# scrose/pylc

Measured on AMD Instinct MI355X. Metric: 512x512 tiles/sec fwd+bwd (DeepLabV3+/ResNet101, 9-class), higher is better.
Workload: dtype f32; 1 GPU; DeepLabV3+ ResNet101 OS16, 3-ch 512x512 tiles, 9 classes, CE+Dice+Focal, clip 0.5 + AdamW, bs=32/GPU (BASELINE.json configs[2]); global_batch=32, parallelism=dp1, conv_arithmetic=f16x3 split (fp32-grade), rccl_ranks=0, wgrad_queue=compute stream, sync_bn=True, activation_format=fp16 planes between BatchNorm and conv kernels (4 B/element)

## Files before the change

### include/pylc_hip.h

```cpp
#ifndef PYLC_HIP_H
#define PYLC_HIP_H

#include <stddef.h>
#include <stdint.h>

#ifdef __cplusplus
extern "C" {
#endif

#define PYLC_OK 0
#define PYLC_ERR_ARG 1
#define PYLC_ERR_HIP 2
#define PYLC_ERR_WORKSPACE 3
#define PYLC_ERR_UNSUPPORTED 4

const char* pylc_last_error(void);
int pylc_abi_version(void);
int pylc_experimental_build(void);
int pylc_init(void);

typedef struct PylcConvDesc {
    int B, H, W;
    int Cin, Cout;
    int R, S;
// ... 85 lines not shown
} PylcBnBack;
size_t pylc_conv2d_dgrad_bn_floats(const PylcConvDesc* d);
int pylc_conv2d_dgrad_bn(const PylcConvDesc* d, const float* dy, const float* w_crsk, float* dx, int accumulate,
                         const float* add_src, const void* add_mask, const PylcBnBack* bn, float* sums_partial, int* sums_rows,
                         void* stream);
#endif
int pylc_relu_bwd_bits(const float* dout, const void* mask, float* g_out, long long M, int C, void* stream);
int pylc_conv2d_dgrad_needs_f32_weights(const PylcConvDesc* d);
size_t pylc_conv2d_wgrad_workspace(const PylcConvDesc* d);
int pylc_conv2d_wgrad(const PylcConvDesc* d, const float* x, const float* dy, float* dw_krsc,
                      float* dbias ,
                      void* workspace, size_t workspace_bytes, void* stream);
typedef struct PylcSlabSum {
    const float* slabs;
    float* dw;
    long long n4;
    long long slab_stride;
    int splits;
    int reserved;
} PylcSlabSum;
int pylc_conv2d_wgrad_slabs(const PylcConvDesc* d, const float* x, const float* dy, float* dw_krsc, void* workspace, size_t workspace_bytes,
                            PylcSlabSum* pending, void* stream);
int pylc_splitk_reduce_batch(const PylcSlabSum* table_dev, const long long* tile_prefix_dev, int n, long long total_tiles, void* stream);
int pylc_weight_transpose(const float* w_krsc, float* w_crsk, int K, int RS, int C, void* stream);

typedef struct PylcDwDesc {
    int B, H, W, C;
    int stride, dil;
    int OH, OW;
    int x_pitch, y_pitch;
} PylcDwDesc;
int pylc_dwconv3x3_fwd(const PylcDwDesc* d, const float* x, const float* w, float* y, void* stream);
int pylc_dwconv3x3_fwd_stats_rows(const PylcDwDesc* d);
int pylc_dwconv3x3_fwd_stats(const PylcDwDesc* d, const float* x, const float* w_c9, float* y, float* stats_partial, void* stream);
int pylc_dwconv3x3_dgrad(const PylcDwDesc* d, const float* dy, const float* w, float* dx, void* stream);
int pylc_dwconv3x3_dgrad_acc(const PylcDwDesc* d, const float* dy, const float* w_c9, float* dx, int accumulate, void* stream);
size_t pylc_dwconv3x3_wgrad_workspace(const PylcDwDesc* d);
int pylc_dwconv3x3_wgrad(const PylcDwDesc* d, const float* x, const float* dy, float* dw,
                         void* workspace, size_t workspace_bytes, void* stream);
int pylc_dwconv3x3_half_ok(const PylcDwDesc* d);
int pylc_dwconv3x3_fwd_h_stats_rows(const PylcDwDesc* d);
int pylc_dwconv3x3_fwd_h(const PylcDwDesc* d, const void* x_h, const unsigned int* x_bound, const float* w_c9, const unsigned int* w_amax,
                         void* y_h, unsigned int* y_bound_out, float* stats_partial, void* stream);
int pylc_dwconv3x3_fwd_h_eval(const PylcDwDesc* d, const void* x_h, const unsigned int* x_bound, const unsigned int* x_true_amax, const float* w,
                              const unsigned int* w_amax, void* y_h, unsigned int* y_bound_out, void* stream);
int pylc_dwconv3x3_dgrad_h(const PylcDwDesc* d, const void* dy_h, const unsigned int* dy_bound, const float* w_c9, const unsigned int* w_amax,
// ... 283 lines not shown
```

### pylc_amd/csrc/conv_common.h

```cpp
#pragma once
#include "common.h"
#include <type_traits>

namespace pylc {

typedef float f32x4 __attribute__((ext_vector_type(4)));
typedef float f32x16 __attribute__((ext_vector_type(16)));

typedef __bf16 bf16x8 __attribute__((ext_vector_type(8)));

typedef _Float16 f16x8 __attribute__((ext_vector_type(8)));
typedef _Float16 f16x2 __attribute__((ext_vector_type(2)));
typedef float f32x2 __attribute__((ext_vector_type(2)));

constexpr int LDB = 80;

__device__ __forceinline__ void split3(const float (&x)[4], uint2& p0, uint2& p1, uint2& p2) {
    unsigned u0[4], u1[4], u2[4];
#pragma unroll
    for (int e = 0; e < 4; ++e) {
        u0[e] = __float_as_uint(x[e]);
        const float r1 = x[e] - __uint_as_float(u0[e] & 0xFFFF0000u);
        u1[e] = __float_as_uint(r1);
        const float r2 = r1 - __uint_as_float(u1[e] & 0xFFFF0000u);
// ... 130 lines not shown
    const unsigned* amax_x;
    long long x_bytes, dy_bytes;
    const void* x_planes;
    const void* dy_planes;
    long long x_plane_stride, dy_plane_stride;
    int nterms;
    int dbg_flags;
};

typedef short s16x4 __attribute__((ext_vector_type(4)));
typedef short s16x8 __attribute__((ext_vector_type(8)));
typedef s16x4 __attribute__((address_space(3))) * lds_s16x4_ptr;

__host__ __device__ constexpr int wg_rowb(int w) { return w * 2 + (w == 32 ? 0 : 64); }

__device__ __forceinline__ bf16x8 tr_frag(const char* p, int rowb) {
    const s16x4 lo = __builtin_amdgcn_ds_read_tr16_b64_v4i16((lds_s16x4_ptr)(p));
    const s16x4 hi = __builtin_amdgcn_ds_read_tr16_b64_v4i16((lds_s16x4_ptr)(p + 4 * rowb));
    const s16x8 v = __builtin_shufflevector(lo, hi, 0, 1, 2, 3, 4, 5, 6, 7);
    return __builtin_bit_cast(bf16x8, v);
}


int launch_wg_pl(WgradArgs& a, int cfg, long long grid, hipStream_t st);
int wgrad_pl_init();

bool takes_pl(const GatherGemmArgs& a);
int launch_gg_pl(GatherGemmArgs& a, hipStream_t st);
int conv_pl_init();
bool takes_stem(const GatherGemmArgs& a);
int launch_stem_fwd(GatherGemmArgs& a, hipStream_t st);
int conv_stem_init();

extern int g_conv_precision;
extern int g_wg_flags;
extern int g_pp_flags;

}
```

### pylc_amd/csrc/conv_igemm.hip

```cpp
#include "conv_common.h"

namespace pylc {

template <int BM, int BN, int WM, int WN, bool CIN4, int PREC>
__global__ __launch_bounds__((BM / WM) * (BN / WN) * 64, 2) void gather_gemm_kernel(const GatherGemmArgs a) {
    constexpr int WAVES_N = BN / WN;
    constexpr int MT = WM / 32, NT = WN / 32;
    constexpr int NTHR = (BM / WM) * (BN / WN) * 64;
    constexpr int RPI = NTHR / 8;
    constexpr int A_IT = BM / RPI, B_IT = BN / RPI;
    static_assert(NTHR == 256 || NTHR == 512, "4 or 8 waves per block");
    static_assert(BM % RPI == 0 && BN % RPI == 0, "tile rows must divide evenly over the loader");
    extern __shared__ __attribute__((aligned(16))) float smem[];
    float* sA = smem;
    float* sB = smem + 2 * BM * LDT;

    const int tile = xcd_remap(blockIdx.x, gridDim.x);
    const int m0 = (tile / a.tiles_n) * BM;
    const int n0 = (tile % a.tiles_n) * BN;
    const int tid = threadIdx.x, lane = tid & 63, wave = tid >> 6;
    const int wave_m = wave / WAVES_N, wave_n = wave % WAVES_N;
    const int v = tid & 7, r0 = tid >> 3;

    int rowh[A_IT], roww[A_IT], rowpix[A_IT];
// ... 1878 lines not shown

extern "C" int pylc_splitk_reduce_batch(const PylcSlabSum* table_dev, const long long* tile_prefix_dev, int n, long long total_tiles, void* stream) {
    PYLC_REQUIRE(table_dev && tile_prefix_dev && n > 0 && total_tiles > 0, "splitk_reduce_batch: bad arguments");
    const int blocks = (int)(total_tiles < 4096 ? total_tiles : 4096);
    hipLaunchKernelGGL(splitk_reduce_batch_kernel, dim3(blocks), dim3(256), 0, as_stream(stream), table_dev, tile_prefix_dev, n, total_tiles);
    PYLC_LAUNCH_CHECK();
    return PYLC_OK;
}

static int wgrad_impl(const PylcConvDesc* d, const float* x, const float* dy, float* dw, float* dbias,
                      void* workspace, size_t workspace_bytes, PylcSlabSum* pending, void* stream);

extern "C" int pylc_conv2d_wgrad(const PylcConvDesc* d, const float* x, const float* dy, float* dw, float* dbias,
                                 void* workspace, size_t workspace_bytes, void* stream) {
    return wgrad_impl(d, x, dy, dw, dbias, workspace, workspace_bytes, nullptr, stream);
}

extern "C" int pylc_conv2d_wgrad_slabs(const PylcConvDesc* d, const float* x, const float* dy, float* dw, void* workspace, size_t workspace_bytes,
                                       PylcSlabSum* pending, void* stream) {
    PYLC_REQUIRE(pending != nullptr, "conv2d_wgrad_slabs: null `pending`");
    return wgrad_impl(d, x, dy, dw, nullptr, workspace, workspace_bytes, pending, stream);
}

static int wgrad_impl(const PylcConvDesc* d, const float* x, const float* dy, float* dw, float* dbias,
                      void* workspace, size_t workspace_bytes, PylcSlabSum* pending, void* stream) {
    if (int rc = check_desc(d)) return rc;
    PYLC_REQUIRE(x && dy && dw, "null pointer");
    PYLC_REQUIRE(dbias == nullptr, "dbias: use pylc_bn_stats on dy (column sums)");
    PYLC_REQUIRE(d->x_fmt == d->dy_fmt, "conv2d_wgrad: x and dy must be in the same format (both fp32 or both fp16 planes; pylc_to_planes converts)");
    hipStream_t st = as_stream(stream);
    const WgradPlan p = plan_wgrad(d);
    const size_t need = p.splits > 1 ? (size_t)p.splits * p.slab * sizeof(float) : 0;
    if (need > workspace_bytes || (need && !workspace))
        return fail(PYLC_ERR_WORKSPACE, "wgrad workspace too small: need %zu bytes, got %zu", need, workspace_bytes);
    PYLC_REQUIRE(p.slab % 4 == 0, "dw size must be a multiple of 4");
    const int T = d->R * d->S;
    WgradArgs a{};
    a.x = x; a.dy = dy; a.out = p.splits > 1 ? static_cast<float*>(workspace) : dw;
    a.P = d->OH; a.Q = d->OW; a.M = d->B * d->OH * d->OW;
    a.IH = d->H; a.IW = d->W; a.Cin = d->Cin; a.x_pitch = d->x_pitch; a.in_sh = a.in_sw = d->stride;
    a.TR = d->R; a.TS = d->S; a.dh0 = -d->pad; a.dh_step = d->dil; a.dw0 = -d->pad; a.dw_step = d->dil;
    a.N = d->Cout; a.N_ld = roundup4(d->Cout); a.dy_pitch = d->y_pitch;
    PYLC_REQUIRE(a.N_ld <= d->y_pitch, "dy pitch must cover roundup4(Cout)");
    a.out_row_stride = T * d->Cin;
    a.tiles_n = p.tiles_n; a.tiles_c = p.tiles_c; a.splits = p.splits; a.m_per_split = p.m_per_split;
    a.slab_stride = p.slab;
    PYLC_REQUIRE(g_conv_precision < 2 || (d->dy_amax && d->x_amax), "f16x3 / fp16 mode: conv2d_wgrad needs dy_amax and x_amax in the descriptor");
    a.x_bytes = (((long long)d->B * d->H * d->W - 1) * d->x_pitch + d->Cin) * 4;
    a.dy_bytes = (((long long)d->B * d->OH * d->OW - 1) * d->y_pitch + a.N_ld) * 4;
    a.amax_dy = d->dy_amax; a.amax_x = d->x_amax;
    const long long grid = (long long)p.tiles_n * p.tiles_c * (p.cin4 ? 1 : T) * p.splits;
    int rc;
    if (d->x_fmt == 1) {
        PYLC_REQUIRE(g_conv_precision >= 2 && !p.cin4 && d->Cout % 8 == 0, "conv2d_wgrad: fp16-plane operands need precision mode 2 or 3, "
                     "a dense geometry and Cout %% 8 == 0");
        a.x_planes = x; a.dy_planes = dy; a.x = nullptr; a.dy = nullptr;
        a.x_plane_stride = planes_stride_rule((long long)d->B * d->H * d->W, d->Cin, d->x_pitch, (g_conv_precision == 3 ? 1 : 2));
        a.dy_plane_stride = planes_stride_rule((long long)d->B * d->OH * d->OW, d->Cout, d->y_pitch, (g_conv_precision == 3 ? 1 : 2));
        a.N_ld = d->Cout;
        a.x_bytes /= 2; a.dy_bytes = (((long long)d->B * d->OH * d->OW - 1) * d->y_pitch + a.N_ld) * 2;
        a.nterms = g_conv_precision == 3 ? 1 : 3;
        rc = launch_wg_pl(a, p.cfg, grid, st);
    } else
    switch (p.cfg) {
        case 0: rc = launch_wg<128, 128, 64, 64, false>(a, grid, st); break;
        case 1: rc = launch_wg<64, 64, 32, 32, false>(a, grid, st); break;
        case 2: rc = launch_wg<32, 128, 32, 32, false>(a, grid, st); break;
        default: rc = launch_wg<64, 64, 32, 32, true>(a, grid, st); break;
    }
    if (rc) return rc;
    if (pending != nullptr) {
        *pending = PylcSlabSum{p.splits > 1 ? static_cast<const float*>(workspace) : nullptr, dw, p.slab / 4, p.slab, p.splits > 1 ? p.splits : 0, 0};
        return PYLC_OK;
    }
    if (p.splits > 1) {
        const long long n4 = p.slab / 4;
        const int blocks = (int)(cdiv<long long>(n4, 32) < 4096 ? cdiv<long long>(n4, 32) : 4096);
        hipLaunchKernelGGL(splitk_reduce_kernel, dim3(blocks), dim3(256), 0, st, static_cast<const float*>(workspace), dw, n4,
                           p.splits, p.slab);
        PYLC_LAUNCH_CHECK();
    }
    return PYLC_OK;
}

extern "C" int pylc_weight_transpose(const float* w, float* wt, int K, int RS, int C, void* stream) {
    PYLC_REQUIRE(w && wt && K > 0 && RS > 0 && C > 0, "bad weight_transpose arguments");
    const int Kp = roundup4(K);
    dim3 grid(cdiv(C, 32), cdiv(Kp, 32), RS);
    hipLaunchKernelGGL(weight_transpose_kernel, grid, dim3(256), 0, as_stream(stream), w, wt, K, RS, C, Kp);
    PYLC_LAUNCH_CHECK();
    return PYLC_OK;
}
```

### pylc_amd/csrc/wgrad_pl.hip

```cpp
#include "conv_common.h"

namespace pylc {

typedef __attribute__((address_space(3))) void* wg_lds_vptr;
template <int BN, int BC, int WN, int WC, int NTERMS, int FAST, bool ACC1 = false, int SETS = 1, bool M16 = false, bool DMA = false>
__global__ __launch_bounds__(256, ACC1 ? 4 : 2) void wgrad_pl_kernel(const WgradArgs a) {
    static_assert(!DMA || (M16 && SETS == 1), "DMA: the 16x16x32 image only");
    constexpr int NPL = NTERMS == 3 ? 2 : 1;
    constexpr int WAVES_C = BC / WC;
    constexpr int NT = WN / 32, CT = WC / 32;
    static_assert(!M16 || (BN == 128 && BC == 128 && WN == 64 && WC == 64 && !ACC1), "M16: 128 x 128 block tiles, 64 x 64 wave tiles, two accumulator sets");
    constexpr int VA = BN / 8, RA = 256 / VA, IA = 32 / RA > 0 ? 32 / RA : 1;
    constexpr int VB = BC / 8, RB = 256 / VB, IB = 32 / RB > 0 ? 32 / RB : 1;
    constexpr bool A_ALL = RA <= 32, B_ALL = RB <= 32;
    constexpr int ROWA = M16 ? 256 : wg_rowb(BN), ROWB = M16 ? 256 : wg_rowb(BC);
    constexpr int PLA = 32 * ROWA, PLB = 32 * ROWB;
    static_assert((BN / WN) * (BC / WC) == 4, "4 waves per block");
    static_assert(FAST == 1 || FAST == 2, "buffer-load geometry paths only");
    extern __shared__ __attribute__((aligned(16))) float smem[];
    char* sA = reinterpret_cast<char*>(smem);
    char* sB = sA + NPL * PLA;
    constexpr int STG = NPL * (PLA + PLB);

    const int T = a.TR * a.TS;
    int id = (a.dbg_flags & 1) ? (int)blockIdx.x : xcd_remap(blockIdx.x, gridDim.x);
    int tc, tn, tap, split;
    if (a.dbg_flags & 2) {
        split = id % a.splits; id /= a.splits;
        tc = id % a.tiles_c; id /= a.tiles_c;
        tn = id % a.tiles_n; id /= a.tiles_n;
        tap = id;
    } else if (a.dbg_flags & 4) {
        tc = id % a.tiles_c; id /= a.tiles_c;
        tn = id % a.tiles_n; id /= a.tiles_n;
        tap = id % T; id /= T;
        split = id;
    } else if (a.Cin > a.N && !(a.dbg_flags & 8)) {
        tap = id % T; id /= T;
        tn = id % a.tiles_n; id /= a.tiles_n;
        tc = id % a.tiles_c; id /= a.tiles_c;
        split = id;
    } else {
        tap = id % T; id /= T;
        tc = id % a.tiles_c; id /= a.tiles_c;
        tn = id % a.tiles_n; id /= a.tiles_n;
        split = id;
    }
    const int n0 = tn * BN, c0 = tc * BC;
// ... 382 lines not shown
                    if (n < a.N) out[(size_t)n * a.out_row_stride + col_base + c] = val;
                }
        }
        return;
    }
#pragma unroll
    for (int j = 0; j < CT; ++j) {
        const int c = c0 + wave_c * WC + j * 32 + (lane & 31);
        if (c >= a.Cin) continue;
#pragma unroll
        for (int i = 0; i < NT; ++i) {
#pragma unroll
            for (int r = 0; r < 16; ++r) {
                const int n = n0 + wave_n * WN + i * 32 + (r & 3) + 8 * (r >> 2) + 4 * (lane >> 5);
                float val = acc[i][j][r];
                if constexpr (TWO_ACC) val = (val + acc_lo[i][j][r] * (1.f / 2048.f)) * unscale_a * unscale_b;
                else val = val * unscale_a * unscale_b;
                if (n < a.N) out[(size_t)n * a.out_row_stride + col_base + c] = val;
            }
        }
    }
}

template <int BN, int BC, int NTERMS>
constexpr size_t wgpl_smem() { return (size_t)(NTERMS == 3 ? 2 : 1) * 32 * (wg_rowb(BN) + wg_rowb(BC)); }

int g_wg_flags = 0;
extern "C" int pylc_debug_wgrad_flags(int flags) { g_wg_flags = flags; return PYLC_OK; }
int g_wg_m16 = 2;
extern "C" int pylc_debug_wgrad_m16(int on) { g_wg_m16 = on; return PYLC_OK; }
int g_wg_dma = 1;
extern "C" int pylc_debug_wgrad_dma(int on) { g_wg_dma = on; return PYLC_OK; }
int g_wg_sets = 1;
extern "C" int pylc_debug_wgrad_sets(int mode) { g_wg_sets = mode; return PYLC_OK; }
int g_wg_acc1 = 0;
extern "C" int pylc_debug_wgrad_acc1(int on) { g_wg_acc1 = on; return PYLC_OK; }
constexpr size_t kAcc1LdsReserve = 72 * 1024;

template <int BN, int BC, int WN, int WC>
static int launch_cfg(const WgradArgs& a, long long grid, hipStream_t st) {
    const int fast = a.Q % 32 == 0 ? 1 : 2;
    const dim3 g((unsigned)grid), b(256);
    if constexpr (BN == 128 && BC == 128) {
        if (a.nterms == 3 && g_wg_acc1) {
            if (fast == 1) hipLaunchKernelGGL((wgrad_pl_kernel<BN, BC, WN, WC, 3, 1, true>), g, b, kAcc1LdsReserve, st, a);
            else hipLaunchKernelGGL((wgrad_pl_kernel<BN, BC, WN, WC, 3, 2, true>), g, b, kAcc1LdsReserve, st, a);
// ... 37 lines not shown
            if (fast == 1) hipLaunchKernelGGL((wgrad_pl_kernel<BN, BC, WN, WC, 3, 1, false, 2>), g, b, lds, st, a);
            else hipLaunchKernelGGL((wgrad_pl_kernel<BN, BC, WN, WC, 3, 2, false, 2>), g, b, lds, st, a);
        } else if (fast == 1) hipLaunchKernelGGL((wgrad_pl_kernel<BN, BC, WN, WC, 3, 1>), g, b, lds, st, a);
        else hipLaunchKernelGGL((wgrad_pl_kernel<BN, BC, WN, WC, 3, 2>), g, b, lds, st, a);
    }
    PYLC_LAUNCH_CHECK();
    return PYLC_OK;
}

int launch_wg_pl(WgradArgs& a, int cfg, long long grid, hipStream_t st) {
    a.dbg_flags = g_wg_flags;
    PYLC_REQUIRE(grid > 0 && grid < (1ll << 31), "wgrad grid out of range");
    PYLC_REQUIRE(a.x_planes && a.dy_planes && a.amax_dy && a.amax_x, "wgrad (fp16-plane operands): null planes / ranges");
    PYLC_REQUIRE(a.Q >= 16 && a.Cin % 8 == 0 && a.N_ld % 8 == 0 && a.x_pitch % 8 == 0 && a.dy_pitch % 8 == 0,
                 "wgrad (fp16-plane operands): needs OW >= 16 and channel counts / pitches that are multiples of 8");
    PYLC_REQUIRE(a.x_bytes < 0xFFFFFFF0ll && a.dy_bytes < 0xFFFFFFF0ll, "wgrad (fp16-plane operands): a plane must stay below 4 GiB");
    switch (cfg) {
        case 0: return launch_cfg<128, 128, 64, 64>(a, grid, st);
        case 1: return launch_cfg<64, 64, 32, 32>(a, grid, st);
        default: return launch_cfg<32, 128, 32, 32>(a, grid, st);
    }
}

template <typename K>
static hipError_t opt_in(K kernel, size_t bytes) {
    return hipFuncSetAttribute(reinterpret_cast<const void*>(kernel), hipFuncAttributeMaxDynamicSharedMemorySize, (int)bytes);
}

int wgrad_pl_init() {
#define PYLC_OPT(BN, BC, WN, WC)                                                                      \
    PYLC_HIP(opt_in(wgrad_pl_kernel<BN, BC, WN, WC, 3, 1>, wgpl_smem<BN, BC, 3>()));                  \
    PYLC_HIP(opt_in(wgrad_pl_kernel<BN, BC, WN, WC, 3, 2>, wgpl_smem<BN, BC, 3>()));                  \
    PYLC_HIP(opt_in(wgrad_pl_kernel<BN, BC, WN, WC, 1, 1>, wgpl_smem<BN, BC, 1>()));                  \
    PYLC_HIP(opt_in(wgrad_pl_kernel<BN, BC, WN, WC, 1, 2>, wgpl_smem<BN, BC, 1>()));                  \
    PYLC_HIP(opt_in((wgrad_pl_kernel<BN, BC, WN, WC, 3, 1, false, 2>), wgpl_smem<BN, BC, 3>()));      \
    PYLC_HIP(opt_in((wgrad_pl_kernel<BN, BC, WN, WC, 3, 2, false, 2>), wgpl_smem<BN, BC, 3>()));      \
    PYLC_HIP(opt_in((wgrad_pl_kernel<BN, BC, WN, WC, 1, 1, false, 2>), wgpl_smem<BN, BC, 1>()));      \
    PYLC_HIP(opt_in((wgrad_pl_kernel<BN, BC, WN, WC, 1, 2, false, 2>), wgpl_smem<BN, BC, 1>()));
    PYLC_OPT(128, 128, 64, 64)
    PYLC_HIP(opt_in((wgrad_pl_kernel<128, 128, 64, 64, 3, 1, false, 1, true, true>), 2 * 4 * 32 * 256));
    PYLC_HIP(opt_in((wgrad_pl_kernel<128, 128, 64, 64, 3, 2, false, 1, true, true>), 2 * 4 * 32 * 256));
    PYLC_HIP(opt_in(wgrad_pl_kernel<128, 128, 64, 64, 3, 1, true>, kAcc1LdsReserve));
    PYLC_HIP(opt_in(wgrad_pl_kernel<128, 128, 64, 64, 3, 2, true>, kAcc1LdsReserve));
    PYLC_OPT(64, 64, 32, 32)
    PYLC_OPT(32, 128, 32, 32)
#undef PYLC_OPT
    return PYLC_OK;
}

}
```

### pylc_amd/lib.py

```python
import ctypes as C
import os

import torch

_HERE = os.path.dirname(os.path.abspath(__file__))
LIB_PATH = os.environ.get('PYLC_LIB') or os.path.join(_HERE, 'libpylc_hip.so')

ABI_VERSION = 15


class PylcError(RuntimeError):
    pass


class ConvDesc(C.Structure):
    _fields_ = [(n, C.c_int) for n in ('B', 'H', 'W', 'Cin', 'Cout', 'R', 'S', 'stride', 'pad', 'dil',
                                       'OH', 'OW', 'x_pitch', 'y_pitch')] + \
               [(n, C.c_void_p) for n in ('x_amax', 'w_amax', 'dy_amax',
                                          'w_planes', 'w_planes_t')] + \
               [(n, C.c_int) for n in ('x_fmt', 'dy_fmt', 'out_fmt')] + [('out_bound', C.c_void_p)] + \
               [('w_planes_fmt', C.c_int)]


class WPrepEntry(C.Structure):
# ... 73 lines not shown
    'pylc_amax': (_I, [_P, _LL, _I, _I, _P, _P]),
    'pylc_amax_segments': (_I, [_P, _P, _I, _P, _P]),
    'pylc_to_planes': (_I, [_P, _I, _P, _I, _LL, _LL, _I, _P, _I, _P]),
    'pylc_from_planes': (_I, [_P, _I, _LL, _P, _I, _LL, _I, _P, _I, _P]),
    'pylc_planes_colsum_workspace_floats': (C.c_size_t, [_I]),
    'pylc_planes_colsum': (_I, [_P, _I, _LL, _I, _P, _LL, _I, _P, _P, _P]),
    'pylc_weight_prepare': (_I, [_P, _P, _I, _LL, _P, _P, _I, _P]),
    'pylc_conv2d_dgrad_needs_f32_weights': (_I, [C.POINTER(ConvDesc)]),
    'pylc_conv2d_fwd': (_I, [C.POINTER(ConvDesc), _P, _P, _P, _P, _P]),
    'pylc_conv2d_fwd_bnact': (_I, [C.POINTER(ConvDesc), _P, _P, _P, _P, _P, _P, _I, _P, _P, _P]),
    'pylc_conv2d_fwd_bnact_ex': (_I, [C.POINTER(ConvDesc), _P, _P, _P, C.POINTER(FwdEp), _P, _P]),
    'pylc_conv2d_fwd_stats_floats': (_SZ, [C.POINTER(ConvDesc)]),
    'pylc_conv2d_fwd_stats': (_I, [C.POINTER(ConvDesc), _P, _P, _P, _P, _P, C.POINTER(_I), _P]),
    'pylc_conv2d_dgrad': (_I, [C.POINTER(ConvDesc), _P, _P, _P, _I, _P]),
    'pylc_conv2d_dgrad_add': (_I, [C.POINTER(ConvDesc), _P, _P, _P, _I, _P, _P, _P]),
    'pylc_relu_bwd_bits': (_I, [_P, _P, _P, _LL, _I, _P]),
    'pylc_conv2d_dgrad_bn_floats': (_SZ, [C.POINTER(ConvDesc)]),
    'pylc_conv2d_dgrad_bn': (_I, [C.POINTER(ConvDesc), _P, _P, _P, _I, _P, _P, C.POINTER(BnBack), _P, C.POINTER(_I), _P]),
    'pylc_bn_bwd_sums_from_partial': (_I, [_P, _I, _I, _P, _P, _P, _D, _P, _P, _P]),
    'pylc_conv2d_wgrad_workspace': (_SZ, [C.POINTER(ConvDesc)]),
    'pylc_conv2d_wgrad': (_I, [C.POINTER(ConvDesc), _P, _P, _P, _P, _P, _SZ, _P]),
    'pylc_conv2d_wgrad_slabs': (_I, [C.POINTER(ConvDesc), _P, _P, _P, _P, _SZ, C.POINTER(SlabSum), _P]),
    'pylc_splitk_reduce_batch': (_I, [_P, _P, _I, C.c_longlong, _P]),
    'pylc_weight_transpose': (_I, [_P, _P, _I, _I, _I, _P]),
    'pylc_dwconv3x3_fwd': (_I, [C.POINTER(DwDesc), _P, _P, _P, _P]),
    'pylc_dwconv3x3_fwd_stats_rows': (_I, [C.POINTER(DwDesc)]),
    'pylc_dwconv3x3_fwd_stats': (_I, [C.POINTER(DwDesc), _P, _P, _P, _P, _P]),
    'pylc_dwconv3x3_dgrad': (_I, [C.POINTER(DwDesc), _P, _P, _P, _P]),
    'pylc_dwconv3x3_dgrad_acc': (_I, [C.POINTER(DwDesc), _P, _P, _P, _I, _P]),
    'pylc_dwconv3x3_wgrad_workspace': (_SZ, [C.POINTER(DwDesc)]),
    'pylc_dwconv3x3_wgrad': (_I, [C.POINTER(DwDesc), _P, _P, _P, _P, _SZ, _P]),
    'pylc_dwconv3x3_half_ok': (_I, [C.POINTER(DwDesc)]),
    'pylc_dwconv3x3_fwd_h_stats_rows': (_I, [C.POINTER(DwDesc)]),
    'pylc_dwconv3x3_bn_ok': (_I, [C.POINTER(DwDesc)]),
    'pylc_dwconv3x3_fwd_h_bn': (_I, [C.POINTER(DwDesc), _P, _P, _P, _P, _I, _P, _P, _P, _P, _P, _P, _P]),
    'pylc_dwconv3x3_wgrad_h_bn': (_I, [C.POINTER(DwDesc), _P, _P, _P, _P, _I, _P, _P, _P, _P, _P, _SZ, _P]),
    'pylc_dwconv3x3_dgrad_h_add_ok': (_I, [C.POINTER(DwDesc)]),
    'pylc_dwconv3x3_dgrad_h_add': (_I, [C.POINTER(DwDesc), _P, _P, _P, _P, _P, _P, _P, _P]),
    'pylc_dwconv3x3_fwd_h': (_I, [C.POINTER(DwDesc), _P, _P, _P, _P, _P, _P, _P, _P]),
    'pylc_dwconv3x3_fwd_h_eval': (_I, [C.POINTER(DwDesc), _P, _P, _P, _P, _P, _P, _P, _P]),
    'pylc_dwconv3x3_dgrad_h': (_I, [C.POINTER(DwDesc), _P, _P, _P, _P, _P, _P, _I, _P, _P]),
    'pylc_dwconv3x3_wgrad_h': (_I, [C.POINTER(DwDesc), _P, _P, _P, _P, _P, _P, _SZ, _P]),
    'pylc_bn_workspace_floats': (_SZ, [_LL, _I]),
    'pylc_bn_stats': (_I, [_P, _LL, _I, _I, _P, _P, _P]),
    'pylc_bn_stats_from_partial': (_I, [_P, _I, _I, _P, _P]),
    'pylc_bn_finalize': (_I, [_P, _D, _I, _P, _P, _F, _F, _I, _P, _P, _P, _P, _P, _P, _P]),
# ... 161 lines not shown
```

### pylc_amd/ops/_core.py

```python
import ctypes as C

import os
import time
from collections import OrderedDict
import torch
import torch.distributed as dist

from .. import lib as L
from ..lib import lib, check, ptr, stream, ConvDesc, DwDesc
from ..runtime import runtime as _runtime


def empty_nhwc(b, c, h, w, device, pitch=None, dtype=torch.float32):
    pitch = c if pitch is None else pitch
    t = torch.empty((b, h, w, pitch), device=device, dtype=dtype).permute(0, 3, 1, 2)
    return t if pitch == c else t[:, :c]


def zeros_nhwc(b, c, h, w, device, pitch=None):
    pitch = c if pitch is None else pitch
    t = torch.zeros((b, h, w, pitch), device=device, dtype=torch.float32).permute(0, 3, 1, 2)
    return t if pitch == c else t[:, :c]


# ... 332 lines not shown
    if not torch.device(device).type == 'cuda':
        return None
    return _side_streams.get(torch.device(device).index)


_side_keep = {}


def _keep_for_side(device, *tensors):
    keep = _side_keep.setdefault(torch.device(device).index, [])
    keep.extend(t for t in tensors if t is not None)
    if len(keep) > 8192:
        sync_side_streams()


_pending_slab_sums = {}
_slab_tables = {}
SLAB_TABLES_MAX = 16


_slab_callback = {}


def add_slab_sum(device, entry):
    idx = torch.device(device).index
    _pending_slab_sums.setdefault(idx, []).append(bytes(entry))
    if idx not in _slab_callback:
        st = torch.cuda.current_stream(idx)

        def at_end_of_backward(idx=idx, st=st):
            _slab_callback.pop(idx, None)
            if _pending_slab_sums.get(idx):
                with torch.cuda.stream(st):
                    flush_slab_sums(torch.device('cuda', idx))
        try:
            torch.autograd.Variable._execution_engine.queue_callback(at_end_of_backward)
            _slab_callback[idx] = st
        except RuntimeError:
            pass


def slab_sum_pending(device, workspace):
    pend = _pending_slab_sums.get(torch.device(device).index)
    if not pend:
        return False
    p = workspace.data_ptr()
    return any(L.SlabSum.from_buffer_copy(e).slabs == p for e in pend)


def reset_slab_sums():
    for pend in _pending_slab_sums.values():
        pend.clear()
    _slab_callback.clear()


def flush_slab_sums(device=None):
    for idx in ([torch.device(device).index] if device is not None else list(_pending_slab_sums)):
        pend = _pending_slab_sums.get(idx)
        if not pend:
            continue
        key = b''.join(pend)
        pend.clear()
        tables = _slab_tables.setdefault(idx, OrderedDict())
        cached = tables.get(key)
        if cached is None:
            n = len(key) // C.sizeof(L.SlabSum)
            ents = (L.SlabSum * n).from_buffer_copy(key)
            prefix = [0]
            for e in ents:
                prefix.append(prefix[-1] + (e.n4 + 31) // 32)
            dev = torch.device('cuda', idx)
            tab_h = torch.frombuffer(bytearray(key), dtype=torch.uint8).pin_memory()
            pre_h = torch.tensor(prefix, dtype=torch.int64).pin_memory()
            cached = tables[key] = (tab_h.to(dev, non_blocking=True), pre_h.to(dev, non_blocking=True), n, prefix[-1], tab_h, pre_h)
            while len(tables) > SLAB_TABLES_MAX:
                tables.popitem(last=False)
        else:
            tables.move_to_end(key)
        with torch.cuda.device(idx):
# ... 163 lines not shown
```

### pylc_amd/ops/conv.py

```python
from . import _core
from ._core import *


def _padded_stem_filter(w, cin):
    arena = getattr(w, '_pylc_arena', None)
    arena = arena() if arena is not None else None
    key = (w._version, arena.generation if arena is not None else -1, cin)
    cache = getattr(w, '_pylc_w4', None)
    if cache is not None and cache[0] == key:
        return cache[1]
    cout, cin_w, r, s = w.shape
    w_k = torch.zeros((cout, r, s, cin), device=w.device, dtype=torch.float32)
    w_k[..., :cin_w] = w.detach().permute(0, 2, 3, 1)
    w._pylc_w4 = (key, w_k)
    return w_k


class Conv2dFn(torch.autograd.Function):

    @staticmethod
    def forward(ctx, x, w, bias, stride, pad, dil, want_stats=False, x_amax=None, w_amax=None, res_link=None, out=None, convert=False, bn_src=None):
        L.init()
        ctx.set_materialize_grads(False)
        ctx.res_link = res_link if (res_link is not None and ctx.needs_input_grad[0]) else None
# ... 192 lines not shown
                mark_planes(dx, dx_bound)
            if link is not None:
                link.pending -= 1
                if link.pending > 0:
                    link.buf, dx = dx, None
                else:
                    link.buf = None
        if ctx.needs_input_grad[1]:
            side = _side_stream(x.device) if _runtime.side_stream_on() else None
            tgt = _grad_target(w)

            def launch_wgrad(side=side, tgt=tgt, x=x, dy=dy, w=w, w_k=w_k, d=d, dy_amax=dy_amax, x_amax=x_amax):
                if side is not None:
                    ev = torch.cuda.Event()
                    ev.record()
                    side.wait_event(ev)
                    _keep_for_side(x.device, x, dy, w_k, dy_amax, x_amax)
                with torch.cuda.stream(side) if side is not None else _nullcontext():
                    sst = stream()
                    nbytes = lib.pylc_conv2d_wgrad_workspace(C.byref(d))
                    ws = _ws(nbytes, x.device)
                    if cin_w % 4 == 0 and tgt is not None and side is None and _runtime.batch_slab_sums and nbytes > 0:
                        own = getattr(w, '_pylc_slab_ws', None)
                        if own is not None and own.is_cuda and _core.slab_sum_pending(own.device, own):
                            _core.flush_slab_sums(own.device)
                        if own is None or own.numel() * 4 < nbytes or own.device != x.device:
                            own = w._pylc_slab_ws = torch.empty(nbytes // 4 + 1, device=x.device)
                        dwl = tgt
                        pend = L.SlabSum()
                        check(lib.pylc_conv2d_wgrad_slabs(C.byref(d), ptr(x), ptr(dy), ptr(dwl), ptr(own), nbytes, C.byref(pend), sst))
                        if pend.splits > 0:
                            _core.add_slab_sum(x.device, pend)
                    elif cin_w % 4 == 0:
                        dwl = tgt if tgt is not None else torch.empty((cout, r, s, cin), device=x.device).permute(0, 3, 1, 2)
                        check(lib.pylc_conv2d_wgrad(C.byref(d), ptr(x), ptr(dy), ptr(dwl), None, ptr(ws), nbytes, sst))
                    else:
                        dw4 = torch.empty((cout, r, s, cin), device=x.device)
                        check(lib.pylc_conv2d_wgrad(C.byref(d), ptr(x), ptr(dy), ptr(dw4), None, ptr(ws), nbytes, sst))
                        dwl = tgt if tgt is not None else torch.empty((cout, r, s, cin_w), device=x.device).permute(0, 3, 1, 2)
                        dwl.copy_(dw4[..., :cin_w].permute(0, 3, 1, 2))
                if side is not None and tgt is None:
                    torch.cuda.current_stream().wait_stream(side)
                return _deliver_grad(w, dwl)

            hold = getattr(w, '_pylc_wgrad_hold', 0) if _runtime.wgrad_hold else 0
            if hold and side is not None and tgt is not None:
                _defer_wgrad(x.device, launch_wgrad, hold)
                dw = None
            elif _runtime.defer_wgrad_1x1 and r * s == 1 and side is not None and tgt is not None:
                _defer_wgrad(x.device, launch_wgrad)
                dw = None
            else:
                dw = launch_wgrad()
        if has_bias and ctx.needs_input_grad[2] and getattr(dy, '_pylc_zero_colsum', False) and _runtime.skip_zero_bias_grad:
            tgt = _grad_target(bias)
            if tgt is not None:
                tgt.zero_()
                db = _deliver_grad(bias, tgt)
            else:
# ... 244 lines not shown
```

### pylc_amd/runtime.py

```python
import itertools
import os


class _Runtime:
    def side_stream_on(self):
        if self.wgrad_side_stream is None:
            from .lib import lib
            return lib.pylc_get_conv_precision() == 3
        return bool(self.wgrad_side_stream)

    def __init__(self):
        self.sync_group = None
        self.sync_bn = os.environ.get('PYLC_SYNC_BN', '1') != '0'
        self.coalesce_sync_bn = True
        self.bn_refine = True
        self.defer_wgrad_1x1 = False
        self.wgrad_hold = True
        self.grad_group = None
        self.grad_ready = None
        self.wgrad_side_stream = False if os.environ.get('PYLC_NO_SIDE_STREAM') else (True if os.environ.get('PYLC_SIDE_STREAM') else None)
        self.wgrad_cus = 0
        self.no_relu_bits = False
        self.fuse_res_grad = True
        self.fuse_proj_bn = True
        self.skip_zero_bias_grad = True
        self.defer_bn_apply = True
        self.upcat_planes = True
        self.fused_grad_ranges = True
        self.gap_planes = True
        self.batch_slab_sums = True
        self.fuse_bn_sums = False
        self.half_acts = True
        self.half_dw = True
        self.eval_planes = True
        self.fuse_eval_bn = True
        self.bn_clamp_eps = False
        self.dropout_enabled = True
        self.no_planes = False
        self.planes_dy = True
        self.pool_planes = True
        self.fold_planes = True
        self.dw_wgrad_side = True
        self.adamw_ranges = True
        self.grad_overlap = True
        self.decoder_hold = (0, 0)
        self.debug_planes = False
        self.debug_streams = False
        self.planes_only = ''
        self.planes_fwd_only = False
        self.comm = None
        self.grad_comm = None
        self.shard_check = None
        self.collectives = 0
# ... 54 lines not shown
```

Measured before the change: 446.3 tiles/s.

## Batch small fp16-plane weight-gradient convs into one grouped kernel launch

```diff
diff --git a/include/pylc_hip.h b/include/pylc_hip.h
--- a/include/pylc_hip.h
+++ b/include/pylc_hip.h
@@ -131,6 +131,11 @@
 int pylc_conv2d_wgrad_slabs(const PylcConvDesc* d, const float* x, const float* dy, float* dw_krsc, void* workspace, size_t workspace_bytes,
                             PylcSlabSum* pending, void* stream);
 int pylc_splitk_reduce_batch(const PylcSlabSum* table_dev, const long long* tile_prefix_dev, int n, long long total_tiles, void* stream);
+int pylc_wgrad_group_max(void);
+long long pylc_conv2d_wgrad_group_blocks(const PylcConvDesc* d);
+int pylc_conv2d_wgrad_slabs_group(const PylcConvDesc* descs, const void* const* x, const void* const* dy, float* const* dw_krsc,
+                                  void* const* workspaces, const size_t* workspace_bytes, PylcSlabSum* pending, int n, int* grouped,
+                                  void* stream);
 int pylc_weight_transpose(const float* w_krsc, float* w_crsk, int K, int RS, int C, void* stream);
 
 typedef struct PylcDwDesc {
diff --git a/pylc_amd/csrc/conv_common.h b/pylc_amd/csrc/conv_common.h
--- a/pylc_amd/csrc/conv_common.h
+++ b/pylc_amd/csrc/conv_common.h
@@ -176,7 +176,20 @@
 }
 
 
+struct WgradGroupEntry {
+    WgradArgs a;
+    int first, blocks;
+};
+constexpr int kWgradGroupMax = 16;
+struct WgradGroupArgs {
+    WgradGroupEntry e[kWgradGroupMax];
+    int n;
+};
+static_assert(sizeof(WgradGroupArgs) <= 4096, "a launch carries at most 4 KB of kernel arguments");
+
 int launch_wg_pl(WgradArgs& a, int cfg, long long grid, hipStream_t st);
+bool wg_pl_groupable(WgradArgs& a, int cfg, long long grid, int* fast);
+int launch_wg_pl_group(const WgradGroupArgs& g, int fast, long long grid, hipStream_t st);
 int wgrad_pl_init();
 
 bool takes_pl(const GatherGemmArgs& a);
diff --git a/pylc_amd/csrc/conv_igemm.hip b/pylc_amd/csrc/conv_igemm.hip
--- a/pylc_amd/csrc/conv_igemm.hip
+++ b/pylc_amd/csrc/conv_igemm.hip
@@ -1924,20 +1924,18 @@
     return wgrad_impl(d, x, dy, dw, nullptr, workspace, workspace_bytes, pending, stream);
 }
 
-static int wgrad_impl(const PylcConvDesc* d, const float* x, const float* dy, float* dw, float* dbias,
-                      void* workspace, size_t workspace_bytes, PylcSlabSum* pending, void* stream) {
+static int wgrad_prepare(const PylcConvDesc* d, const float* x, const float* dy, float* dw, void* workspace, size_t workspace_bytes,
+                         WgradPlan& p, WgradArgs& a, long long& grid) {
     if (int rc = check_desc(d)) return rc;
     PYLC_REQUIRE(x && dy && dw, "null pointer");
-    PYLC_REQUIRE(dbias == nullptr, "dbias: use pylc_bn_stats on dy (column sums)");
     PYLC_REQUIRE(d->x_fmt == d->dy_fmt, "conv2d_wgrad: x and dy must be in the same format (both fp32 or both fp16 planes; pylc_to_planes converts)");
-    hipStream_t st = as_stream(stream);
-    const WgradPlan p = plan_wgrad(d);
+    p = plan_wgrad(d);
     const size_t need = p.splits > 1 ? (size_t)p.splits * p.slab * sizeof(float) : 0;
     if (need > workspace_bytes || (need && !workspace))
         return fail(PYLC_ERR_WORKSPACE, "wgrad workspace too small: need %zu bytes, got %zu", need, workspace_bytes);
     PYLC_REQUIRE(p.slab % 4 == 0, "dw size must be a multiple of 4");
     const int T = d->R * d->S;
-    WgradArgs a{};
+    a = WgradArgs{};
     a.x = x; a.dy = dy; a.out = p.splits > 1 ? static_cast<float*>(workspace) : dw;
     a.P = d->OH; a.Q = d->OW; a.M = d->B * d->OH * d->OW;
     a.IH = d->H; a.IW = d->W; a.Cin = d->Cin; a.x_pitch = d->x_pitch; a.in_sh = a.in_sw = d->stride;
@@ -1951,8 +1949,7 @@
     a.x_bytes = (((long long)d->B * d->H * d->W - 1) * d->x_pitch + d->Cin) * 4;
     a.dy_bytes = (((long long)d->B * d->OH * d->OW - 1) * d->y_pitch + a.N_ld) * 4;
     a.amax_dy = d->dy_amax; a.amax_x = d->x_amax;
-    const long long grid = (long long)p.tiles_n * p.tiles_c * (p.cin4 ? 1 : T) * p.splits;
-    int rc;
+    grid = (long long)p.tiles_n * p.tiles_c * (p.cin4 ? 1 : T) * p.splits;
     if (d->x_fmt == 1) {
         PYLC_REQUIRE(g_conv_precision >= 2 && !p.cin4 && d->Cout % 8 == 0, "conv2d_wgrad: fp16-plane operands need precision mode 2 or 3, "
                      "a dense geometry and Cout %% 8 == 0");
@@ -1962,8 +1959,27 @@
         a.N_ld = d->Cout;
         a.x_bytes /= 2; a.dy_bytes = (((long long)d->B * d->OH * d->OW - 1) * d->y_pitch + a.N_ld) * 2;
         a.nterms = g_conv_precision == 3 ? 1 : 3;
-        rc = launch_wg_pl(a, p.cfg, grid, st);
-    } else
+    }
+    return PYLC_OK;
+}
+
+static PylcSlabSum slab_sum_of(const WgradPlan& p, float* dw, void* workspace) {
+    return PylcSlabSum{p.splits > 1 ? static_cast<const float*>(workspace) : nullptr, dw, p.slab / 4, p.slab, p.splits > 1 ? p.splits : 0, 0};
+}
+
+static int wgrad_impl(const PylcConvDesc* d, const float* x, const float* dy, float* dw, float* dbias,
+                      void* workspace, size_t workspace_bytes, PylcSlabSum* pending, void* stream) {
+    if (int rc = check_desc(d)) return rc;
+    PYLC_REQUIRE(x && dy && dw, "null pointer");
+    PYLC_REQUIRE(dbias == nullptr, "dbias: use pylc_bn_stats on dy (column sums)");
+    hipStream_t st = as_stream(stream);
+    WgradPlan p;
+    WgradArgs a;
+    long long grid;
+    if (int rc = wgrad_prepare(d, x, dy, dw, workspace, workspace_bytes, p, a, grid)) return rc;
+    int rc;
+    if (d->x_fmt == 1) rc = launch_wg_pl(a, p.cfg, grid, st);
+    else
     switch (p.cfg) {
         case 0: rc = launch_wg<128, 128, 64, 64, false>(a, grid, st); break;
         case 1: rc = launch_wg<64, 64, 32, 32, false>(a, grid, st); break;
@@ -1972,7 +1988,7 @@
     }
     if (rc) return rc;
     if (pending != nullptr) {
-        *pending = PylcSlabSum{p.splits > 1 ? static_cast<const float*>(workspace) : nullptr, dw, p.slab / 4, p.slab, p.splits > 1 ? p.splits : 0, 0};
+        *pending = slab_sum_of(p, dw, workspace);
         return PYLC_OK;
     }
     if (p.splits > 1) {
@@ -1982,6 +1998,60 @@
                            p.splits, p.slab);
         PYLC_LAUNCH_CHECK();
     }
+    return PYLC_OK;
+}
+
+extern "C" int pylc_wgrad_group_max(void) { return kWgradGroupMax; }
+
+extern "C" long long pylc_conv2d_wgrad_group_blocks(const PylcConvDesc* d) {
+    if (d == nullptr || d->x_fmt != 1 || d->dy_fmt != 1 || check_desc(d)) return 0;
+    if (g_conv_precision < 2 || !d->dy_amax || !d->x_amax || d->Cout % 8 != 0 || roundup4(d->Cout) > d->y_pitch) return 0;
+    WgradPlan p;
+    WgradArgs a;
+    long long grid;
+    int fast;
+    float* const any = reinterpret_cast<float*>(sizeof(float));
+    if (wgrad_prepare(d, any, any, any, any, ~(size_t)0, p, a, grid)) return 0;
+    return wg_pl_groupable(a, p.cfg, grid, &fast) ? grid : 0;
+}
+
+extern "C" int pylc_conv2d_wgrad_slabs_group(const PylcConvDesc* descs, const void* const* x, const void* const* dy, float* const* dw,
+                                             void* const* workspaces, const size_t* workspace_bytes, PylcSlabSum* pending, int n, int* grouped,
+                                             void* stream) {
+    PYLC_REQUIRE(descs && x && dy && dw && workspaces && workspace_bytes && pending && grouped, "conv2d_wgrad_slabs_group: null argument");
+    PYLC_REQUIRE(n > 0 && n <= kWgradGroupMax, "conv2d_wgrad_slabs_group: 1 .. 16 problems per call");
+    hipStream_t st = as_stream(stream);
+    WgradGroupArgs g[2];
+    std::memset(g, 0, sizeof(g));
+    long long tot[2] = {0, 0};
+    bool single[kWgradGroupMax];
+    for (int i = 0; i < n; ++i) {
+        WgradPlan p;
+        WgradArgs a;
+        long long grid;
+        if (int rc = wgrad_prepare(descs + i, static_cast<const float*>(x[i]), static_cast<const float*>(dy[i]), dw[i], workspaces[i],
+                                   workspace_bytes[i], p, a, grid))
+            return rc;
+        pending[i] = slab_sum_of(p, dw[i], workspaces[i]);
+        int fast = 0;
+        single[i] = !(descs[i].x_fmt == 1 && wg_pl_groupable(a, p.cfg, grid, &fast));
+        if (single[i]) continue;
+        const int f = fast - 1;
+        WgradGroupEntry& e = g[f].e[g[f].n++];
+        e.a = a;
+        e.first = (int)tot[f];
+        e.blocks = (int)grid;
+        tot[f] += (grid + 7) / 8 * 8;
+    }
+    for (int f = 0; f < 2; ++f)
+        if (g[f].n)
+            if (int rc = launch_wg_pl_group(g[f], f + 1, tot[f], st)) return rc;
+    for (int i = 0; i < n; ++i)
+        if (single[i])
+            if (int rc = wgrad_impl(descs + i, static_cast<const float*>(x[i]), static_cast<const float*>(dy[i]), dw[i], nullptr, workspaces[i],
+                                    workspace_bytes[i], pending + i, stream))
+                return rc;
+    *grouped = g[0].n + g[1].n;
     return PYLC_OK;
 }
 
diff --git a/pylc_amd/csrc/wgrad_pl.hip b/pylc_amd/csrc/wgrad_pl.hip
--- a/pylc_amd/csrc/wgrad_pl.hip
+++ b/pylc_amd/csrc/wgrad_pl.hip
@@ -4,7 +4,7 @@
 
 typedef __attribute__((address_space(3))) void* wg_lds_vptr;
 template <int BN, int BC, int WN, int WC, int NTERMS, int FAST, bool ACC1 = false, int SETS = 1, bool M16 = false, bool DMA = false>
-__global__ __launch_bounds__(256, ACC1 ? 4 : 2) void wgrad_pl_kernel(const WgradArgs a) {
+__device__ __forceinline__ void wgrad_pl_body(const WgradArgs& a, const int bid, const int nblk) {
     static_assert(!DMA || (M16 && SETS == 1), "DMA: the 16x16x32 image only");
     constexpr int NPL = NTERMS == 3 ? 2 : 1;
     constexpr int WAVES_C = BC / WC;
@@ -23,7 +23,7 @@
     constexpr int STG = NPL * (PLA + PLB);
 
     const int T = a.TR * a.TS;
-    int id = (a.dbg_flags & 1) ? (int)blockIdx.x : xcd_remap(blockIdx.x, gridDim.x);
+    int id = (a.dbg_flags & 1) ? bid : xcd_remap(bid, nblk);
     int tc, tn, tap, split;
     if (a.dbg_flags & 2) {
         split = id % a.splits; id /= a.splits;
@@ -452,6 +452,22 @@
     }
 }
 
+template <int BN, int BC, int WN, int WC, int NTERMS, int FAST, bool ACC1 = false, int SETS = 1, bool M16 = false, bool DMA = false>
+__global__ __launch_bounds__(256, ACC1 ? 4 : 2) void wgrad_pl_kernel(const WgradArgs a) {
+    wgrad_pl_body<BN, BC, WN, WC, NTERMS, FAST, ACC1, SETS, M16, DMA>(a, (int)blockIdx.x, (int)gridDim.x);
+}
+
+template <int FAST>
+__global__ __launch_bounds__(256, 2) void wgrad_pl_group_kernel(const WgradGroupArgs g) {
+    const int b = (int)blockIdx.x;
+    int e = 0;
+    for (int i = 1; i < g.n; ++i) e = g.e[i].first <= b ? i : e;
+    const int local = b - g.e[e].first, nblk = g.e[e].blocks;
+    if (local >= nblk) return;
+    const WgradArgs a = g.e[e].a;
+    wgrad_pl_body<128, 128, 64, 64, 3, FAST, false, 1, true, true>(a, local, nblk);
+}
+
 template <int BN, int BC, int NTERMS>
 constexpr size_t wgpl_smem() { return (size_t)(NTERMS == 3 ? 2 : 1) * 32 * (wg_rowb(BN) + wg_rowb(BC)); }
 
@@ -535,6 +551,24 @@
     }
 }
 
+bool wg_pl_groupable(WgradArgs& a, int cfg, long long grid, int* fast) {
+    a.dbg_flags = g_wg_flags;
+    *fast = a.Q % 32 == 0 ? 1 : 2;
+    return cfg == 0 && a.nterms == 3 && !g_wg_acc1 && g_wg_dma && (g_wg_m16 == 2 || (g_wg_m16 == 1 && a.TR * a.TS == 1)) &&
+           grid > 0 && grid < (1ll << 24) && a.x_planes && a.dy_planes && a.amax_dy && a.amax_x &&
+           a.Q >= 16 && a.Cin % 8 == 0 && a.N_ld % 8 == 0 && a.x_pitch % 8 == 0 && a.dy_pitch % 8 == 0 &&
+           a.x_bytes < 0xFFFFFFF0ll && a.dy_bytes < 0xFFFFFFF0ll;
+}
+
+int launch_wg_pl_group(const WgradGroupArgs& g, int fast, long long grid, hipStream_t st) {
+    PYLC_REQUIRE(g.n > 0 && g.n <= kWgradGroupMax && grid > 0 && grid < (1ll << 31) && (fast == 1 || fast == 2), "grouped wgrad: bad entries / grid");
+    constexpr size_t lds = 2 * 4 * 32 * 256;
+    if (fast == 1) hipLaunchKernelGGL(wgrad_pl_group_kernel<1>, dim3((unsigned)grid), dim3(256), lds, st, g);
+    else hipLaunchKernelGGL(wgrad_pl_group_kernel<2>, dim3((unsigned)grid), dim3(256), lds, st, g);
+    PYLC_LAUNCH_CHECK();
+    return PYLC_OK;
+}
+
 template <typename K>
 static hipError_t opt_in(K kernel, size_t bytes) {
     return hipFuncSetAttribute(reinterpret_cast<const void*>(kernel), hipFuncAttributeMaxDynamicSharedMemorySize, (int)bytes);
@@ -553,6 +587,8 @@
     PYLC_OPT(128, 128, 64, 64)
     PYLC_HIP(opt_in((wgrad_pl_kernel<128, 128, 64, 64, 3, 1, false, 1, true, true>), 2 * 4 * 32 * 256));
     PYLC_HIP(opt_in((wgrad_pl_kernel<128, 128, 64, 64, 3, 2, false, 1, true, true>), 2 * 4 * 32 * 256));
+    PYLC_HIP(opt_in(wgrad_pl_group_kernel<1>, 2 * 4 * 32 * 256));
+    PYLC_HIP(opt_in(wgrad_pl_group_kernel<2>, 2 * 4 * 32 * 256));
     PYLC_HIP(opt_in(wgrad_pl_kernel<128, 128, 64, 64, 3, 1, true>, kAcc1LdsReserve));
     PYLC_HIP(opt_in(wgrad_pl_kernel<128, 128, 64, 64, 3, 2, true>, kAcc1LdsReserve));
     PYLC_OPT(64, 64, 32, 32)
diff --git a/pylc_amd/lib.py b/pylc_amd/lib.py
--- a/pylc_amd/lib.py
+++ b/pylc_amd/lib.py
@@ -119,6 +119,9 @@
     'pylc_conv2d_wgrad': (_I, [C.POINTER(ConvDesc), _P, _P, _P, _P, _P, _SZ, _P]),
     'pylc_conv2d_wgrad_slabs': (_I, [C.POINTER(ConvDesc), _P, _P, _P, _P, _SZ, C.POINTER(SlabSum), _P]),
     'pylc_splitk_reduce_batch': (_I, [_P, _P, _I, C.c_longlong, _P]),
+    'pylc_wgrad_group_max': (_I, []),
+    'pylc_conv2d_wgrad_group_blocks': (_LL, [C.POINTER(ConvDesc)]),
+    'pylc_conv2d_wgrad_slabs_group': (_I, [C.POINTER(ConvDesc), _P, _P, _P, _P, _P, C.POINTER(SlabSum), _I, C.POINTER(_I), _P]),
     'pylc_weight_transpose': (_I, [_P, _P, _I, _I, _I, _P]),
     'pylc_dwconv3x3_fwd': (_I, [C.POINTER(DwDesc), _P, _P, _P, _P]),
     'pylc_dwconv3x3_fwd_stats_rows': (_I, [C.POINTER(DwDesc)]),
diff --git a/pylc_amd/ops/_core.py b/pylc_amd/ops/_core.py
--- a/pylc_amd/ops/_core.py
+++ b/pylc_amd/ops/_core.py
@@ -378,22 +378,78 @@
 _slab_callback = {}
 
 
+_wgrad_group = {}
+
+
+def _queue_slab_callback(idx):
+    if idx in _slab_callback:
+        return
+    st = torch.cuda.current_stream(idx)
+
+    def at_end_of_backward(idx=idx, st=st):
+        try:
+            if _pending_slab_sums.get(idx) or _wgrad_group.get(idx):
+                with torch.cuda.stream(st):
+                    flush_slab_sums(torch.device('cuda', idx))
+        finally:
+            _slab_callback.pop(idx, None)
+    try:
+        torch.autograd.Variable._execution_engine.queue_callback(at_end_of_backward)
+        _slab_callback[idx] = st
+    except RuntimeError:
+        pass
+
+
+def wgrad_group_blocks(d):
+    if _runtime.wgrad_group <= 1:
+        return 0
+    blocks = lib.pylc_conv2d_wgrad_group_blocks(C.byref(d))
+    return blocks if blocks <= _runtime.wgrad_group_max_blocks else 0
+
+
+def wgrad_noted(device, workspace):
+    grp = _wgrad_group.get(torch.device(device).index)
+    return bool(grp) and any(it[4] is workspace or it[4].data_ptr() == workspace.data_ptr() for it in grp)
+
+
+def note_wgrad(device, d, x, dy, dw, workspace, nbytes, keep=()):
+    idx = torch.device(device).index
+    grp = _wgrad_group.setdefault(idx, [])
+    grp.append((d, x, dy, dw, workspace, nbytes, keep))
+    _queue_slab_callback(idx)
+    if len(grp) >= min(_runtime.wgrad_group, lib.pylc_wgrad_group_max()):
+        flush_wgrad_group(device)
+
+
+def flush_wgrad_group(device=None):
+    for idx in ([torch.device(device).index] if device is not None else list(_wgrad_group)):
+        grp = _wgrad_group.get(idx)
+        if not grp:
+            continue
+        items = list(grp)
+        grp.clear()
+        n = len(items)
+        descs = (L.ConvDesc * n)(*[it[0] for it in items])
+        arrs = [(C.c_void_p * n)(*[ptr(it[k]) for it in items]) for k in (1, 2, 3, 4)]
+        sizes = (C.c_size_t * n)(*[it[5] for it in items])
+        pend = (L.SlabSum * n)()
+        grouped = C.c_int(0)
+        with torch.cuda.device(idx):
+            check(lib.pylc_conv2d_wgrad_slabs_group(descs, arrs[0], arrs[1], arrs[2], arrs[3], sizes, pend, n, C.byref(grouped), stream()))
+        wgrad_group_launches[0] += 1
+        wgrad_group_launches[1] += grouped.value
+        for e in pend:
+            if e.splits > 0:
+                add_slab_sum(torch.device('cuda', idx), e)
+
+
+wgrad_group_launches = [0, 0]
+
+
 def add_slab_sum(device, entry):
     idx = torch.device(device).index
     _pending_slab_sums.setdefault(idx, []).append(bytes(entry))
-    if idx not in _slab_callback:
-        st = torch.cuda.current_stream(idx)
-
-        def at_end_of_backward(idx=idx, st=st):
-            _slab_callback.pop(idx, None)
-            if _pending_slab_sums.get(idx):
-                with torch.cuda.stream(st):
-                    flush_slab_sums(torch.device('cuda', idx))
-        try:
-            torch.autograd.Variable._execution_engine.queue_callback(at_end_of_backward)
-            _slab_callback[idx] = st
-        except RuntimeError:
-            pass
+    _queue_slab_callback(idx)
 
 
 def slab_sum_pending(device, workspace):
@@ -407,10 +463,13 @@
 def reset_slab_sums():
     for pend in _pending_slab_sums.values():
         pend.clear()
+    for grp in _wgrad_group.values():
+        grp.clear()
     _slab_callback.clear()
 
 
 def flush_slab_sums(device=None):
+    flush_wgrad_group(device)
     for idx in ([torch.device(device).index] if device is not None else list(_pending_slab_sums)):
         pend = _pending_slab_sums.get(idx)
         if not pend:
diff --git a/pylc_amd/ops/conv.py b/pylc_amd/ops/conv.py
--- a/pylc_amd/ops/conv.py
+++ b/pylc_amd/ops/conv.py
@@ -238,19 +238,25 @@
                     ws = _ws(nbytes, x.device)
                     if cin_w % 4 == 0 and tgt is not None and side is None and _runtime.batch_slab_sums and nbytes > 0:
                         own = getattr(w, '_pylc_slab_ws', None)
-                        if own is not None and own.is_cuda and _core.slab_sum_pending(own.device, own):
+                        if own is not None and own.is_cuda and (_core.slab_sum_pending(own.device, own) or _core.wgrad_noted(own.device, own)):
                             _core.flush_slab_sums(own.device)
                         if own is None or own.numel() * 4 < nbytes or own.device != x.device:
                             own = w._pylc_slab_ws = torch.empty(nbytes // 4 + 1, device=x.device)
                         dwl = tgt
-                        pend = L.SlabSum()
-                        check(lib.pylc_conv2d_wgrad_slabs(C.byref(d), ptr(x), ptr(dy), ptr(dwl), ptr(own), nbytes, C.byref(pend), sst))
-                        if pend.splits > 0:
-                            _core.add_slab_sum(x.device, pend)
+                        if _core.wgrad_group_blocks(d):
+                            _core.note_wgrad(x.device, d, x, dy, dwl, own, nbytes, (dy_amax, x_amax, w_k))
+                        else:
+                            _core.flush_wgrad_group(x.device)
+                            pend = L.SlabSum()
+                            check(lib.pylc_conv2d_wgrad_slabs(C.byref(d), ptr(x), ptr(dy), ptr(dwl), ptr(own), nbytes, C.byref(pend), sst))
+                            if pend.splits > 0:
+                                _core.add_slab_sum(x.device, pend)
                     elif cin_w % 4 == 0:
+                        _core.flush_wgrad_group(x.device)
                         dwl = tgt if tgt is not None else torch.empty((cout, r, s, cin), device=x.device).permute(0, 3, 1, 2)
                         check(lib.pylc_conv2d_wgrad(C.byref(d), ptr(x), ptr(dy), ptr(dwl), None, ptr(ws), nbytes, sst))
                     else:
+                        _core.flush_wgrad_group(x.device)
                         dw4 = torch.empty((cout, r, s, cin), device=x.device)
                         check(lib.pylc_conv2d_wgrad(C.byref(d), ptr(x), ptr(dy), ptr(dw4), None, ptr(ws), nbytes, sst))
                         dwl = tgt if tgt is not None else torch.empty((cout, r, s, cin_w), device=x.device).permute(0, 3, 1, 2)
diff --git a/pylc_amd/runtime.py b/pylc_amd/runtime.py
--- a/pylc_amd/runtime.py
+++ b/pylc_amd/runtime.py
@@ -29,6 +29,8 @@
         self.fused_grad_ranges = True
         self.gap_planes = True
         self.batch_slab_sums = True
+        self.wgrad_group = 6
+        self.wgrad_group_max_blocks = 1024
         self.fuse_bn_sums = False
         self.half_acts = True
         self.half_dw = True
```

Measured after the change: 448.1 tiles/s, median of 6. Within noise of the previous version (+0.4%).
